# conanhujinming/flash_hash_join

Hardware: AMD Instinct MI355X
Metric: probe throughput (billion probes/sec), int64 keys, whole join (build + probe phases) per step (higher is better)
Workload: dtype int64

## Files before the change

flash_hash_join_amd/api.py:

```python
from __future__ import annotations

import ctypes
import threading
from typing import Any, Dict, Optional, Tuple

import numpy as np

from . import _lib
from ._lib import FjTimings, check

ALGO_ADAPTIVE, ALGO_SCALAR, ALGO_RADIX = 0, 1, 2
ALGO_MANY_TO_MANY = 0x10
ALGO_LEFT_OUTER = 0x20
ALGO_ANTI = 0x40
ALGO_ROW_IDS = 0x80
ALGO_FULL_OUTER = 0x100
ALGO_ALL_COPIES = 0x200
ALGO_PROBE_ORDER = 0x800
ALGO_BUILD_ORDER = 0x1000
ALGO_AGG_MIN = 0x4000
ALGO_AGG_MAX = 0x8000
ALGO_AGG_SIGNED = 0x10000
ALGO_GROUP_BY = 0x40000
ALGO_INVERSE = 0x100000
# ... 77 lines not shown
    return _ctxs[device]


def workspace_bytes(device: Optional[int] = None) -> int:
    L = _lib.load()
    return sum(int(L.fj_ctx_workspace_bytes(h)) for d, h in _ctxs.items() if device is None or d == device)


def trim_workspace(device: Optional[int] = None) -> None:
    L = _lib.load()
    for d, h in list(_ctxs.items()):
        if device is None or d == device:
            with _ctx_locks.setdefault(d, threading.RLock()):
                check(L.fj_ctx_trim(h))
    check(L.fj_ctx_trim(None))


def set_option(name: str, value: int) -> None:
    check(_lib.load().fj_set_option(name.encode(), int(value)))


def get_option(name: str) -> int:
    v = int(_lib.load().fj_get_option(name.encode()))
    if v < 0:
        raise KeyError(_lib.last_error())
    return v


def last_timings() -> Optional[dict]:
    return _last.as_dict() if _last is not None else None


def _join_host(algo: int, bloom: int, materialize: int, bk, bv, pk, return_arrays: bool):
    global _last
    L = _lib.load()
    bk, pk = _as_u64_host(bk, "build_keys"), _as_u64_host(pk, "probe_keys")
    bv = _as_u64_host(bv, "build_values") if bv is not None else None
    if bv is not None and bv.size < bk.size:
        raise ValueError(f"build_values has {bv.size} elements, build_keys has {bk.size}")
    cnt = (ctypes.c_uint64 * 3)(0, 0, 0)
    sec = ctypes.c_double(0.0)
    ok, ov = ctypes.c_void_p(), ctypes.c_void_p()
    want = bool(materialize and return_arrays)
    check(L.fj_join_host(algo, bloom, materialize, bk.ctypes.data, bv.ctypes.data if bv is not None else None, bk.size, pk.ctypes.data, pk.size,
                         cnt, ctypes.byref(sec),
                         ctypes.byref(ok) if want else None, ctypes.byref(ov) if want else None))
    t = FjTimings()
# ... 1567 lines not shown
```

flash_hash_join_amd/csrc/fj_host.h:

```cpp
#pragma once
#include "fj_internal.h"
#include "../../include/flashjoin.h"
#include "../../include/flashjoin_lab.h"

#include <algorithm>
#include <chrono>
#include <cstdarg>
#include <cstdio>
#include <cstdlib>
#include <cstring>
#include <condition_variable>
#include <functional>
#include <mutex>
#include <string>
#include <thread>
#include <vector>

struct StreamState;

namespace fjh {

int set_err(const char* fmt, ...);
fj_timings& last_timings();
#define HIPCHK(x)                                                                                          \
// ... 83 lines not shown
struct Plan { int bits = 0, npass = 0; int fan_log[4] = {0, 0, 0, 0}; int bloom_level = 0; };

struct Prepared {
    enum Form { EMPTY, LDS, HBM };
    bool valid = false;
    Form form = EMPTY;
    bool has_vals = false;
    int top_bits = 64, path = 0;
    Plan plan; u32 nparts = 0;
    size_t nb = 0; u64 g = 0;
    u64* keys = nullptr; u64* rows = nullptr; u64* vals = nullptr; void* aux = nullptr;
    u64 cap_mask = 0;
    size_t bytes = 0;
};

struct PassIter {
    int side = 0; bool has_vals = false; size_t n = 0; Plan plan; int used = 64; u32 parents = 1; u64 lbound = 0;
    u32 tile_chunks = 16; int i = 0;
    FjChunkSet prev{}; bool have_prev = false; const uint4* tiles = nullptr; const u32* ntiles = nullptr; const u32* toff = nullptr;
    FjChunkSet cs{}; u32 Gmax = 1, F = 1, appends = 1;
    size_t piece_rows = 0;
    int slot = 0, cs_base = 0;
    u32 item_tc_max = 0;
    bool want_items = false; u32 items_cap = 0; u32* part_count = nullptr; int part_count_slot = W_PART_COUNT;
    bool bloom_done = false; const FjChunkSet* bloom_build = nullptr;
    const u32* bloom_prebuilt = nullptr;
    unsigned long long* bloom_bucket_keys = nullptr;
    int save_level = 0; FjChunkSet saved{};
    u32* alloc_word = nullptr; u32* seg_word = nullptr; u32* err_word = nullptr;
    bool in_pk7 = false; u32 in_b0 = 0, in_top_shift = 0;
    bool vals_pos = false;
};

}

struct PackState {
    bool begun = false, deferred = false;
    u32 part_shift = 0;
    fjh::PassIter it;
    FjPackArgs args{};
    int nranks = 0;
};

struct StreamState {
    bool active = false;
    fjh::Plan plan; fjh::PassIter pit, bit; FjLdsJoinArgs ja{};
// ... 37 lines not shown
    u32 reserve_cus = 0;
    void* stage[3] = {nullptr, nullptr, nullptr};
    size_t stage_bytes = 0;
    bool plan_in_flight = false;
    bool slot_dirty[fjh::W_NSLOTS] = {};
    std::recursive_mutex mu;
};

namespace fjh {

#define FJ_HOOK_LOOPBACK 1
#define FJ_HOOK_INJECT_FAIL 2
#define FJ_HOOK_SPLIT_ALWAYS 4
#define FJ_HOOK_ONE_COMM 8
#define FJ_HOOK_RESERVE_ALWAYS 16
#define FJ_HOOK_EMIT_TAGGED 32
#define FJ_HOOK_EMIT_RETRY_7TH 64
struct Options {
    size_t radix_threshold = 0; int scalar_hbm_table = 0; u32 persistent_min_items = 8192; u32 plan_target_keys = FJ_PART_TARGET_KEYS;
    int bloom_variant = 0, bloom_auto = 1, bloom_auto_max_hit_bp = 2300, mat_single_pass = 1;
    int join_wide = 2;
    u32 lab_hooks = 0;
    u32 join_items_target = 2048;
    int mm_heavy_keys = 0;
    int mm_heavy_outer = 0;
    Options();
};
Options& options();

int get_buf(fj_ctx* c, int slot, size_t bytes, void** out);
int get_zeroed_buf(fj_ctx* c, int slot, size_t bytes, void** out, hipStream_t s);
int plan_npass(int bits);
void plan_passes(Plan& p, bool extra_first);
Plan make_plan(size_t nb, int top_bits, bool want_bloom = false, u64 target_override = 0);
void pass_init(PassIter& it, int side, bool has_vals, size_t n, const Plan& plan, int top_bits);
u32 pass_groups(u64 chunks, u64 rows, u32 tile_chunks, u32 F);
int pass_prepare(fj_ctx* c, PassIter& it, u32 appends, hipStream_t s);
int pass_launch(fj_ctx* c, PassIter& it, const u64* keys, const u64* vals, size_t n, hipStream_t s, int* ev_cursor);
bool bloom_stage_follows(const PassIter& it, int level);
void join_item_geometry(u64 nparts, size_t np, u64 chunk_bound, u32* tc, u64* max_items);
bool wide_join_planned(bool materialize, size_t nb, size_t np_eff, int bits);
int level_finish(fj_ctx* c, PassIter& it, bool final_level, hipStream_t s);
int pass_complete(fj_ctx* c, PassIter& it, hipStream_t s);
int bloom_stage(fj_ctx* c, PassIter& it, hipStream_t s);
int run_passes(fj_ctx* c, PassIter& it, const u64* keys, const u64* vals, hipStream_t s, FjChunkSet* out, int* ev_cursor);
int clear_plan_scalars(fj_ctx* c, hipStream_t s);
void begin_plan(fj_ctx* c);
void end_plan(fj_ctx* c);
void drop_pending(fj_ctx* c);
int begin_step(fj_ctx* c, const char* who);
int read_scalars(fj_ctx* c, hipStream_t s);
float ev_ms(fj_ctx* c, int a, int b);
void plan_timings(fj_ctx* c, const Plan& plan, u64 partitions, int evc, fj_timings* t);
int stamps_begin(unsigned long long** dbg, hipStream_t s);
int stamps_report(const char* label, const unsigned long long* dbg, u32 nitems, hipStream_t s);

int emit_pending(fj_ctx* c, u64* d_ok, u64* d_ov, size_t cap, hipStream_t s, fj_timings* t);
int radix_join_tail(fj_ctx* c, int materialize, FjLdsJoinArgs& ja, const Plan& plan, size_t np, const PassIter& pit, hipStream_t s,
                    fj_timings* t, int evc, u64* out_count, bool* lds_full, int top_bits, SingleOut* so = nullptr);

int join_outer(fj_ctx* c, int mode, bool use_radix, const u64* bk, const u64* bv, size_t nb, const u64* pk, size_t np, int top_bits,
               hipStream_t s, fj_timings* t, u64* out_count, u64* d_ok, u64* d_ov, bool rid = false);
int join_full(fj_ctx* c, bool use_radix, const u64* bk, const u64* bv, size_t nb, const u64* pk, size_t np, int top_bits,
// ... 36 lines not shown
```

flash_hash_join_amd/csrc/fj_internal.h:

```cpp
#pragma once
#include "fj_common.h"

#define FJ_ERR_POOL 1u
#define FJ_ERR_LDS_FULL 2u
#define FJ_STAT_DUPS 4u
#define FJ_STAT_RETRY 8u
#define FJ_STAT_EMIT_RETRY 16u
#define FJ_ERR_VARIANT 32u
#define FJ_BLOOM_HDR_MAGIC 0xB100F000u
#define FJ_STAT_TOOBIG 64u
#define FJ_ERR_OUTCAP 128u
#define FJ_ITEM_RETRY 0xFFFFFFFFu
#define FJ_ITEM_TOOBIG 0xFFFFFFFEu

struct FjPartArgs {
    const u64* in_keys;
    const u64* in_vals;
    const u32* in_list;
    const u32* in_dir;
    const uint4* in_tiles;
    const u32* in_ntiles;
    u64 n_flat;
    u32 parent0;
    u64* out_keys;
// ... 94 lines not shown
    u32 nsplit;
    const uint4* items;
    const u32* nitems_dev;
    u32 items_cap;
    u32* part_count;
    unsigned long long* total;
    u32* err;
    const u64* out_off;
    u64* out_keys;
    u64* out_vals;
    unsigned long long* out_cursor;
    u64 out_capacity;
    u32 retry_only;
    u32 mark_toobig;
    u32 want_dups;
    u32 dedup;
    const u64* orig_vals;
    u32 avg_build_keys;
    unsigned long long* dbg;
    u32 dbg_flags;
    u32 row_ids;
};
hipError_t fj_launch_lds_join(const FjLdsJoinArgs& a, bool materialize, hipStream_t s, u32* next_item = nullptr,
                              u32 persistent_min_items = 8192);
hipError_t fj_launch_emit_single(const FjLdsJoinArgs& a, hipStream_t s, u32* next_item);
#define FJ_WIDE_MAXSRC 16u
struct FjWideArgs {
    const u32* toff; u32 part_lo, part_hi;
    const unsigned char* base; u32 nsrc, bits, mid_bytes;
    u32 group_log;
    u32 max_units;
    u32 pmask;
    u64 offs_off[FJ_WIDE_MAXSRC], lo_off[FJ_WIDE_MAXSRC], mid_off[FJ_WIDE_MAXSRC];
};
hipError_t fj_launch_count_join_wide(const FjLdsJoinArgs& a, const FjWideArgs& w, bool dense, u32 grid, hipStream_t s);
static inline u32 fj_wide_pmask(int bits, int top_bits) { return bits <= 0 ? 0u : (bits >= 32 ? 0xFFFFFFFFu : ((1u << bits) - 1u) << (top_bits - 32 - bits)); }

hipError_t fj_launch_lds_join_retry(const FjLdsJoinArgs& a, hipStream_t s);
hipError_t fj_launch_lds_emit_retry(const FjLdsJoinArgs& a, hipStream_t s, bool only_marked = true);

hipError_t fj_launch_sample_hits(const FjChunkSet& build, const u64* pk, u64 np, u32 nsamples, u32 shift32, u32 pmask,
                                 unsigned long long* hits, hipStream_t s);

#define FJ_MM_INNER 0
#define FJ_MM_LEFT 1
#define FJ_MM_FULL 2
struct FjMmOuterArgs {
// ... 152 lines not shown
```

flash_hash_join_amd/csrc/fj_join.hip:

```cpp
#include "fj_lds_table_dev.h"

namespace {

constexpr u32 S = FJ_LDS_SLOTS;

struct JoinHdr {
    u32 cnt, has_empty, cursor, claimed, full, ovf;
    u32 pad[2];
    u64 empty_val;
    u64 pad2;
};

constexpr u32 NGRP = S / FJ_LDS_GROUP;
__device__ __forceinline__ void lds_groups(u64 key, u32& g1, u32& g2) {
    const u32 w = FJ_HW2(key);
    g1 = (w & (NGRP - 1)) * FJ_LDS_GROUP;
    g2 = ((w >> 11) & (NGRP - 1)) * FJ_LDS_GROUP;
}

__device__ __forceinline__ u32 lds_tag(u32 w2) { const u32 t = w2 >> 24; return t ? t : 1u; }
__device__ __forceinline__ u32 tag_zero_bytes(u32 t) {
    const u32 y = (t & 0x7F7F7F7Fu) + 0x7F7F7F7Fu;
    return ~(y | t | 0x7F7F7F7Fu);
}
// ... 784 lines not shown
                            const u64 ok = __ballot((okm >> (h + i)) & 1u);
                            wave_hits += (u32)__popcll(ok & ((hit & ~ise) | (ise & he)));
                        }
                    }
                    if (!parked) park();
                }
            }
        }
        if (!parked) park();
        if (lane == 0 && wave_hits) atomicAdd(&hdr->cnt, wave_hits);
        __syncthreads();
        if (lvn) load_build(bmn, 0, nbbn); else bok = 0;
        if (tid == 0) {
            const u32 cnt = (lv && !full) ? hdr->cnt : 0u;
            if (full) atomicOr(a.err, FJ_STAT_RETRY);
            a.part_count[d.item] = full ? FJ_ITEM_RETRY : cnt;
            if (cnt) atomicAdd(a.total, (unsigned long long)cnt);
        }
        if (dn.item >= nitems) break;
        __syncthreads();
        reset_table();
        __syncthreads();
        d = dn; buf ^= 1;
    }
}

struct EkHdr { u32 has_empty, nstash, full, dups, cursor, novf, cur2[2]; u64 empty_val; u64 gb2[2]; u64 pad; u64 stash[CK_STASH]; u64 stash_val[CK_STASH]; };

template <int NT, bool DEDUP, bool SINGLE = false, bool RID = false>
__global__ __launch_bounds__(NT, 4) void fj_emit_join_persistent(FjLdsJoinArgs a, u32* __restrict__ next_item) {
    static_assert(!(SINGLE && DEDUP), "the single-pass form serves unique build keys");
    extern __shared__ __attribute__((aligned(16))) unsigned char smem[];
    EkHdr* hdr = reinterpret_cast<EkHdr*>(smem);
    u64* tkeys = reinterpret_cast<u64*>(smem + sizeof(EkHdr));
    u64* tvals = tkeys + S;
    u32* pm0 = reinterpret_cast<u32*>(tvals + S);
    u32* bm0 = pm0 + 2 * JP_META;
    u32* s_next = bm0 + 2 * JB_META;
    u32* bits = s_next + 4;
    u64* ovf = reinterpret_cast<u64*>(bits + S / 32);
    u32 tid = threadIdx.x;
    const u32 lane = tid & 63, wave_s = (u32)__builtin_amdgcn_readfirstlane((int)(threadIdx.x >> 6));
    auto fresh_tid = [&]() -> u32 {
        u32 t;
        asm volatile("v_mbcnt_lo_u32_b32 %0, -1, 0\n\tv_mbcnt_hi_u32_b32 %0, -1, %0\n\tv_lshl_add_u32 %0, %1, 6, %0" : "=&v"(t) : "s"(wave_s));
        return t;
// ... 811 lines not shown
    const u64 stride = (u64)gridDim.x * blockDim.x;
    for (u64 i = (u64)blockIdx.x * blockDim.x + threadIdx.x; i < n; i += stride) {
        keys[i] = (first + i + 1) * FJ_GOLDEN;
        vals[i] = first + i;
    }
}
__global__ void fj_gen_probe_kernel(u64* __restrict__ keys, u64 first, u64 n, u64 B, u64 seed, u32 hit_bp,
                                    unsigned long long* __restrict__ expected) {
    const u64 stride = (u64)gridDim.x * blockDim.x;
    u32 hits = 0;
    for (u64 i = (u64)blockIdx.x * blockDim.x + threadIdx.x; i < n; i += stride) {
        const u64 j = first + i;
        const u64 r = 1 + fj_mix(seed, j) % B;
        const bool hit = (fj_mix(seed ^ 1ull, j) % 10000ull) < hit_bp;
        keys[i] = (r + (hit ? 0ull : B)) * FJ_GOLDEN;
        hits += hit ? 1u : 0u;
    }
    hits = fj_wave_sum(hits);
    if ((threadIdx.x & 63) == 0 && hits) atomicAdd(expected, (unsigned long long)hits);
}

}

hipError_t fj_launch_lds_join(const FjLdsJoinArgs& a, bool materialize, hipStream_t s, u32* next_item, u32 persistent_min_items) {
    const u32 nb = a.items ? a.items_cap : a.nparts * a.nsplit;
    if (materialize) {
        if (a.row_ids && (!a.dedup || a.orig_vals)) return hipErrorInvalidValue;
        if (a.build.list && a.probe.list && a.items && next_item && nb >= persistent_min_items && !a.dbg && !(a.dbg_flags & ~8u)) {
            const u32 ldsp = sizeof(EkHdr) + 2 * S * 8 + 2 * (JP_META + JB_META) * 4 + 16 + S / 8 + CK_OVF * 8;
            auto pk = a.row_ids ? fj_emit_join_persistent<1024, true, false, true>
                                : a.dedup ? fj_emit_join_persistent<1024, true> : fj_emit_join_persistent<1024, false>;
            hipError_t e = fj_set_max_lds_once(reinterpret_cast<const void*>(pk), ldsp);
            if (e != hipSuccess) return e;
            const u32 grid = nb < 256 ? nb : 256;
            hipLaunchKernelGGL(pk, dim3(grid), dim3(1024), ldsp, s, a, next_item);
            return hipGetLastError();
        }
        if (a.row_ids) return fj_launch_lds_emit_retry(a, s, false);
        const u32 lds = sizeof(JoinHdr) + 2 * S * 8 + S + S / 2 + (JP_META + JB_META) * 4;
        auto kern = (a.build.list && a.probe.list) ? fj_lds_join_kernel<true, 1024, true> : fj_lds_join_kernel<true, 1024, false>;
        hipError_t e = fj_set_max_lds_once(reinterpret_cast<const void*>(kern), lds);
        if (e != hipSuccess) return e;
        hipLaunchKernelGGL(kern, dim3(nb), dim3(1024), lds, s, a);
    } else {
        const u32 lds = sizeof(CkHdr) + S * 8 + (JP_META + JB_META) * 4 + S / 8 + CK_OVF * 8;
        const bool lists = a.build.list && a.probe.list;
        if (lists && next_item && nb >= persistent_min_items && !a.dbg && !a.dbg_flags) {
            const u32 ldsp = sizeof(CkHdr) + S * 8 + 2 * (JP_META + JB_META) * 4 + 16 + S / 8 + CK_OVF * 8;
            auto pk = fj_count_join_persistent<512>;
            hipError_t e = fj_set_max_lds_once(reinterpret_cast<const void*>(pk), ldsp);
            if (e != hipSuccess) return e;
            const u32 grid = nb < 512 ? nb : 512;
            hipLaunchKernelGGL(pk, dim3(grid), dim3(512), ldsp, s, a, next_item);
            return hipGetLastError();
        }
        auto kern = lists ? fj_count_join_kernel<512, true> : fj_count_join_kernel<512, false>;
        hipError_t e = fj_set_max_lds_once(reinterpret_cast<const void*>(kern), lds);
        if (e != hipSuccess) return e;
        hipLaunchKernelGGL(kern, dim3(nb), dim3(512), lds, s, a);
    }
    return hipGetLastError();
}

hipError_t fj_launch_emit_single(const FjLdsJoinArgs& a, hipStream_t s, u32* next_item) {
    if (!a.build.list || !a.probe.list || !a.items || !next_item || !a.out_cursor || a.dedup || !a.build.vals || (a.row_ids && !a.probe.vals))
        return hipErrorInvalidValue;
    const u32 nb = a.items_cap;
    const u32 ldsp = sizeof(EkHdr) + 2 * S * 8 + 2 * (JP_META + JB_META) * 4 + 16 + S / 8 + CK_OVF * 8;
    auto pk = a.row_ids ? fj_emit_join_persistent<1024, false, true, true> : fj_emit_join_persistent<1024, false, true>;
// ... 154 lines not shown
```

flash_hash_join_amd/csrc/fj_joins.hip:

```cpp
#include "fj_host.h"

namespace fjh {

static int skew_side(fj_ctx* c, PassIter& it, int side, bool vals, const FjChunkSet& in, const std::vector<u32>& off, u64 chunks, int S, int bits_left,
                     int slot, int tiles_slot, u32* d_nt, hipStream_t s);

int emit_pending(fj_ctx* c, u64* d_ok, u64* d_ov, size_t cap, hipStream_t s, fj_timings* t) {
    Pending& pd = c->pend;
    if (!pd.valid) return set_err("fj_emit_pairs: no counted materialising join is pending on this context");
    if (pd.count > cap) return set_err("fj_emit_pairs: output capacity %zu < %llu pairs", cap, (unsigned long long)pd.count);
    if (pd.count > 0 && (((uintptr_t)d_ok | (uintptr_t)d_ov) & 7)) return set_err("output buffers must be 8-byte aligned");
    HIPCHK(hipEventRecord(c->ev[E_EMIT0], s));
    if (pd.count > 0) {
        void* p;
        if (pd.kind == Pending::LDS) {
            if (pd.lds.row_ids) {
                pd.lds.dedup = 1; pd.lds.orig_vals = nullptr;
            } else if (pd.has_dups) {
                if (get_buf(c, W_ROWIDX, pd.nb * 8, &p)) return 1;
                u64* rowidx = (u64*)p;
                HIPCHK(fj_launch_iota(rowidx, pd.nb, s));
                HIPCHK(hipMemsetAsync(&c->d_sc->alloc[0], 0, sizeof(c->d_sc->alloc) + sizeof(c->d_sc->seg_counter), s));
                PassIter bit;
                pass_init(bit, 0, true, pd.nb, make_plan(pd.nb, pd.top_bits), pd.top_bits);
// ... 316 lines not shown
        const u32 grid = std::min<u32>(nitems, c->num_cus);
        HIPCHK(fj_launch_count_join_wide(jw, wa, false, grid, s));
        if (jw.dbg) {
            std::vector<unsigned long long> h(4096 * 8);
            HIPCHK(hipStreamSynchronize(s));
            HIPCHK(hipMemcpy(h.data(), jw.dbg, h.size() * 8, hipMemcpyDeviceToHost));
            double acc[8] = {0, 0, 0, 0, 0, 0, 0, 0};
            for (u32 g = 0; g < grid && g < 4096; ++g) for (int i = 0; i < 8; ++i) acc[i] += (double)h[g * 8 + i] * 0.01;
            u32 nit = 0;
            HIPCHK(hipMemcpy(&nit, jw.nitems_dev, 4, hipMemcpyDeviceToHost));
            const double per = (double)std::min<u32>(grid, 4096) * ((double)nit / grid);
            fprintf(stderr, "[FJ_WIDE_STAMPS] us per item (thread 0): rotate+requests %.3f  claim_issue+zero %.3f  barB %.3f  probe %.3f  resolve+park %.3f  barA %.3f  stores %.3f\n",
                    acc[0] / per, acc[5] / per, acc[6] / per, acc[1] / per, acc[2] / per, acc[3] / per, acc[4] / per);
            for (int ph = 0; ph < 3; ++ph) {
                fprintf(stderr, "[FJ_WIDE_STAMPS] wave 0..15, %s:", ph == 0 ? "requests + claims issued + probe" : ph == 1 ? "claims resolved + park (to barrier A)" : "stores (barrier A to B)");
                for (int w = 0; w < 16; ++w) {
                    double sacc = 0;
                    for (u32 g = 0; g < grid && g < 256; ++g) sacc += (double)h[2048 * 8 + g * 64 + w * 4 + ph] * 0.01;
                    fprintf(stderr, " %.2f", sacc / ((double)std::min<u32>(grid, 256) * ((double)nit / grid)));
                }
                fprintf(stderr, "\n");
            }
        }
    } else
    HIPCHK(fj_launch_lds_join(ja, false, s, &c->d_sc->next_item, options().persistent_min_items));
    if (ja.dbg) { if (stamps_report("FJ_JOIN_STAMPS", ja.dbg, nitems, s)) return 1; ja.dbg = nullptr; }
    HIPCHK(hipEventRecord(c->ev[E_JOIN], s));
    if (read_scalars(c, s)) return 1;
    t->lds_retries = 0;
    if ((c->h_sc->err & FJ_STAT_RETRY) && !(c->h_sc->err & (FJ_ERR_POOL | FJ_ERR_LDS_FULL))) {
        ja.retry_only = 1; ja.mark_toobig = ja.items ? 1u : 0u;
        HIPCHK(fj_launch_lds_join_retry(ja, s));
        ja.retry_only = 0;
        HIPCHK(hipEventRecord(c->ev[E_JOIN], s));
        if (read_scalars(c, s)) return 1;
        t->lds_retries = 1;
        if ((c->h_sc->err & FJ_STAT_TOOBIG) && !(c->h_sc->err & (FJ_ERR_POOL | FJ_ERR_LDS_FULL))) {
            bool ok = false; u32 redone = 0;
            if (skew_join(c, ja, plan, top_bits, nitems, pit.slot, materialize, s, &ok, &redone, &c->pend)) return 1;
            HIPCHK(hipEventRecord(c->ev[E_JOIN], s));
            if (read_scalars(c, s)) return 1;
            if (ok) t->lds_retries = 1 + (int)redone;
            else c->h_sc->err |= FJ_ERR_LDS_FULL;
        }
    }
    if (c->h_sc->err & FJ_ERR_POOL) return set_err("internal error: chunk pool exhausted during a partition pass");
    end_plan(c);
    plan_timings(c, plan, ja.nparts, evc, t);
// ... 22 lines not shown
    pass_init(bit, 0, materialize != 0, nb, plan, top_bits);
    bit.vals_pos = rid;
    int evc = 0;
    if (plan.bloom_level > 0) bit.save_level = plan.bloom_level;
    if (run_passes(c, bit, bk, (materialize && !rid) ? bv : nullptr, s, &ja.build, nullptr)) return 1;
    HIPCHK(hipEventRecord(c->ev[E_BUILD], s));
    Plan pplan = plan;
    if (bloom == 2) {
        const u32 nsamp = FJ_SAMPLE_KEYS;
        HIPCHK(fj_launch_sample_hits(ja.build, pk, np, nsamp, (u32)(top_bits - 32 - plan.bits), (1u << plan.bits) - 1u, &c->d_sc->sample_hits, s));
        HIPCHK(hipMemcpyAsync(&c->h_sc->sample_hits, &c->d_sc->sample_hits, sizeof(unsigned long long), hipMemcpyDeviceToHost, s));
        HIPCHK(hipStreamSynchronize(s));
        const u32 hit_bp = (u32)(c->h_sc->sample_hits * 10000ull / nsamp);
        t->sampled_hit_bp = (int)hit_bp;
        if (hit_bp > (u32)options().bloom_auto_max_hit_bp) { pplan = make_plan(nb, top_bits, false); plan.bloom_level = 0; plan.npass = pplan.npass; }
    }
    pass_init(pit, 1, rid, np, pplan, top_bits);
    pit.vals_pos = rid;
    pit.want_items = true;
    {
        size_t np_eff = np;
        if (plan.bloom_level > 0) np_eff = (size_t)((double)np * (t->sampled_hit_bp >= 0 ? std::min(10000, t->sampled_hit_bp + 1000) : 1500) / 10000.0);
        if (wide_join_planned(materialize != 0, nb, np_eff, plan.bits)) pit.item_tc_max = 32;
    }
    if (plan.bloom_level > 0) pit.bloom_build = &bit.saved;
    if (run_passes(c, pit, pk, nullptr, s, &ja.probe, &evc)) return 1;
    HIPCHK(hipEventRecord(c->ev[E_PPART], s));
    ja.avg_build_keys = (u32)std::min<u64>(0xFFFFFFFFu, (u64)nb >> plan.bits);
    ja.row_ids = rid ? 1u : 0u;
    if (radix_join_tail(c, materialize, ja, plan, np, pit, s, t, evc, out_count, lds_full, top_bits, so)) return 1;
    if (c->pend.valid) { c->pend.bk = bk; c->pend.bv = bv; c->pend.nb = nb; c->pend.top_bits = top_bits; }
    return 0;
}

static int mm_tile_join(fj_ctx* c, const FjLdsJoinArgs& ja, u32 nitems, int materialize, hipStream_t s, Pending* pend,
                        int outer = FJ_MM_INNER, const FjMmOuterArgs* oa = nullptr) {
    u32 nlive = 0;
    std::vector<u32> pc(nitems), boff((size_t)ja.build.nb + 1);
    std::vector<uint4> items(nitems);
    HIPCHK(hipMemcpyAsync(&nlive, ja.nitems_dev, 4, hipMemcpyDeviceToHost, s));
    HIPCHK(hipMemcpyAsync(pc.data(), ja.part_count, (size_t)nitems * 4, hipMemcpyDeviceToHost, s));
    HIPCHK(hipMemcpyAsync(items.data(), ja.items, (size_t)nitems * sizeof(uint4), hipMemcpyDeviceToHost, s));
    HIPCHK(hipMemcpyAsync(boff.data(), ja.build.boff, boff.size() * 4, hipMemcpyDeviceToHost, s));
    HIPCHK(hipStreamSynchronize(s));
    if (nlive > nitems) nlive = nitems;
    std::vector<uint4> tiles, big;
// ... 586 lines not shown
```

flash_hash_join_amd/csrc/fj_plan.hip:

```cpp
#include "fj_host.h"

namespace fjh {

namespace { thread_local std::string g_err; thread_local fj_timings g_last; }

int set_err(const char* fmt, ...) {
    char buf[1024];
    va_list ap; va_start(ap, fmt); vsnprintf(buf, sizeof buf, fmt, ap); va_end(ap);
    g_err = buf;
    return 1;
}
fj_timings& last_timings() { return g_last; }

Options& options() { static Options o; return o; }
static int set_option_value(Options& o, const char* name, long long value);
Options::Options() {
    static const char* const legacy[] = {"FJ_RADIX_THRESHOLD", "FJ_SCALAR_HBM_TABLE", "FJ_BLOOM_AUTO", "FJ_BLOOM_AUTO_MAX_HIT_BP", "FJ_BLOOM_VARIANT", "FJ_PLAN_TARGET_KEYS",
                                         "FJ_MAT_SINGLE_PASS", "FJ_PERSISTENT_MIN_ITEMS", "FJ_JOIN_ITEMS_TARGET", "FJ_JOIN_WIDE", "FJ_DIST_LOOPBACK", "FJ_DIST_INJECT_FAIL",
                                         "FJ_DIST_RESERVE_ALWAYS", "FJ_DIST_SPLIT_ALWAYS", "FJ_DIST_ONE_COMM", "FJ_EMIT_TAGGED"};
    for (const char* name : legacy)
        if (getenv(name)) fprintf(stderr, "flash_hash_join_amd: the environment variable %s is no longer read (use FJ_OPTIONS=\"name=value,...\" or fj_set_option; see include/flashjoin.h)\n", name);
    const char* e = getenv("FJ_OPTIONS");
    if (!e) return;
    std::string str(e);
// ... 129 lines not shown
        a.in_keys = it.prev.keys; a.in_vals = it.prev.vals; a.in_list = it.prev.list; a.in_dir = it.prev.dir;
        a.in_tiles = it.tiles; a.in_ntiles = it.ntiles; a.n_flat = 0;
    } else {
        a.in_keys = keys; a.in_vals = vals; a.in_list = nullptr; a.in_dir = nullptr; a.in_tiles = nullptr; a.in_ntiles = nullptr; a.n_flat = n;
        a.vals_pos = it.has_vals && it.vals_pos ? 1u : 0u;
        G = std::min(G, pass_groups((n + FJ_CHUNK - 1) / FJ_CHUNK, n, it.tile_chunks, it.F));
    }
    a.parent0 = 0;
    a.out_keys = cs.keys; a.out_vals = cs.vals; a.out_dir = cs.dir; a.out_rel = cs.rel; a.seg_off = cs.seg_off;
    a.bchunks = cs.bchunks; a.alloc = cs.alloc; a.seg_counter = it.seg_word ? it.seg_word : &c->d_sc->seg_counter[it.side * 4 + it.i];
    a.cap_chunks = cs.cap; a.max_segs = cs.max_segs;
    a.err = it.err_word ? it.err_word : &c->d_sc->err;
    if (it.have_prev && it.in_pk7) { a.in_pk7 = 1; a.in_b0 = it.in_b0; a.in_top_shift = it.in_top_shift; }
    a.shift = (u32)it.used; a.fan_log = (u32)it.plan.fan_log[it.i]; a.slab = fj_slab_for(it.appends); a.run_log = cs.run_log; a.side = (u32)it.side;
    const int line_log = (it.has_vals && it.F > 256) ? 3 : 4;
    if (ev_cursor) HIPCHK(hipEventRecord(c->ev[E_PK0 + 2 * (*ev_cursor)], s));
    HIPCHK(fj_launch_partition(a, it.has_vals, line_log, G, s));
    if (ev_cursor) { HIPCHK(hipEventRecord(c->ev[E_PK0 + 2 * (*ev_cursor) + 1], s)); ++*ev_cursor; }
    return 0;
}

bool bloom_stage_follows(const PassIter& it, int level) { return it.plan.bloom_level == level && it.bloom_build && !it.bloom_done; }

void join_item_geometry(u64 nparts, size_t np, u64 chunk_bound, u32* tc, u64* max_items) {
    const u64 pchunks = (np + FJ_CHUNK - 1) / FJ_CHUNK;
    const u64 bound = std::max<u64>(chunk_bound, pchunks);
    const u64 avg = std::max<u64>(1, bound / nparts);
    u64 want = 1;
    const u64 target_items = options().join_items_target;
    if (nparts < target_items) want = std::min<u64>((target_items + nparts - 1) / nparts, std::max<u64>(1, (pchunks / nparts) / 32));
    *tc = (u32)(want > 1 ? std::max<u64>(8, (avg * 9 / 8 + want - 1) / want) : std::max<u64>(512, 4 * avg));
    *max_items = bound / *tc + nparts + 1;
}

bool wide_join_planned(bool materialize, size_t nb, size_t np_eff, int bits) {
    if (materialize || bits <= 0 || options().join_wide == 0) return false;
    if (options().join_wide == 1) return true;
    return np_eff <= 3 * nb;
}

int level_finish(fj_ctx* c, PassIter& it, bool final_level, hipStream_t s) {
    const FjChunkSet& cs = it.cs;
    u32 tc = 0; u64 max_tiles = 0; u32* zero_tail = nullptr;
    if (bloom_stage_follows(it, it.i)) tc = fj_bloom_tile_chunks();
    else if (!final_level) tc = fj_partition_tile_chunks((u32)it.plan.fan_log[it.i], it.has_vals);
    else if (it.want_items) {
        join_item_geometry(cs.nb, it.n, it.lbound, &tc, &max_tiles);
        if (it.item_tc_max && tc > it.item_tc_max) { tc = it.item_tc_max; max_tiles = std::max<u64>(it.lbound, (it.n + FJ_CHUNK - 1) / FJ_CHUNK) / tc + cs.nb + 1; }
    }
    if (tc && !max_tiles) max_tiles = it.lbound / tc + cs.nb + 1;
    if (max_tiles >= (1ull << 31)) return set_err("internal error: tile table too large");
    u32* toff = nullptr; uint4* tiles = nullptr;
    void* p;
    if (tc) {
        if (get_buf(c, it.cs_base + W_TOFF, ((size_t)cs.nb + 1) * 4, &p)) return 1; toff = (u32*)p;
        if (get_buf(c, it.cs_base + W_TILES, max_tiles * sizeof(uint4), &p)) return 1; tiles = (uint4*)p;
        if (final_level) {
            if (get_buf(c, it.part_count_slot, (size_t)max_tiles * 4, &p)) return 1;
            it.part_count = zero_tail = (u32*)p; it.items_cap = (u32)max_tiles;
        }
    }
    HIPCHK(fj_launch_group(cs, tc, toff, tiles, (u32)max_tiles, zero_tail, s));
    it.tiles = tiles; it.ntiles = toff ? toff + cs.nb : nullptr; it.toff = toff;
    return 0;
}

int pass_complete(fj_ctx* c, PassIter& it, hipStream_t s) {
    const FjChunkSet& cs = it.cs;
    it.lbound = it.n / FJ_CHUNK + 1 + (u64)(it.Gmax + it.parents) * it.F * it.appends;
    ++it.i;
// ... 116 lines not shown
        for (int j = 1; j <= 5; ++j) acc[j] += (double)(r[j] - r[j - 1]) * 0.01;
        if (r[0] < tmin) tmin = r[0];
        if (r[5] > tmax) tmax = r[5];
        ++n;
    }
    if (n == 0) n = 1;
    fprintf(stderr, "[%s] items=%d  meta+init=%.2f  build=%.2f  buildsync=%.2f  probe=%.2f  fin=%.2f us (means); first 4096 items span %.1f us\n",
            label, n, acc[1] / n, acc[2] / n, acc[3] / n, acc[4] / n, acc[5] / n, (double)(tmax - tmin) * 0.01);
    return 0;
}

static int set_option_value(Options& o, const char* name, long long value) {
    if (!strcmp(name, "radix_threshold")) { if (value < 0) return set_err("fj_set_option: radix_threshold must be >= 0"); o.radix_threshold = (size_t)value; return 0; }
    if (!strcmp(name, "scalar_hbm_table")) { o.scalar_hbm_table = value != 0; return 0; }
    if (!strcmp(name, "plan_target_keys")) { if (value < 16 || value > (long long)FJ_PART_TARGET_KEYS) return set_err("fj_set_option: plan_target_keys must be 16..%u", FJ_PART_TARGET_KEYS); o.plan_target_keys = (u32)value; return 0; }
    if (!strcmp(name, "bloom_auto")) { o.bloom_auto = value != 0; return 0; }
    if (!strcmp(name, "mat_single_pass")) { o.mat_single_pass = value != 0; return 0; }
    if (!strcmp(name, "bloom_auto_max_hit_bp")) { if (value < 0 || value > 10000) return set_err("fj_set_option: bloom_auto_max_hit_bp must be 0..10000"); o.bloom_auto_max_hit_bp = (int)value; return 0; }
    if (!strcmp(name, "bloom_variant")) { if (value < 0 || value > 2) return set_err("fj_set_option: bloom_variant must be 0..2"); o.bloom_variant = (int)value; return 0; }
    if (!strcmp(name, "join_wide")) { if (value < 0 || value > 2) return set_err("fj_set_option: join_wide must be 0..2"); o.join_wide = (int)value; return 0; }
    if (!strcmp(name, "persistent_min_items")) { if (value < 0) return set_err("fj_set_option: persistent_min_items must be >= 0"); o.persistent_min_items = (u32)std::min<long long>(value, 0xFFFFFFFFll); return 0; }
    if (!strcmp(name, "lab_hooks")) { if (value < 0 || value > 0xFFFF) return set_err("fj_set_option: lab_hooks is a mask of FJ_HOOK_* bits"); o.lab_hooks = (u32)value; return 0; }
    if (!strcmp(name, "join_items_target")) { if (value < 1 || value > (1 << 20)) return set_err("fj_set_option: join_items_target must be 1..1048576"); o.join_items_target = (u32)value; return 0; }
    if (!strcmp(name, "mm_heavy_keys")) { if (value < 0 || value > 1) return set_err("fj_set_option: mm_heavy_keys must be 0 or 1"); o.mm_heavy_keys = (int)value; return 0; }
    if (!strcmp(name, "mm_heavy_outer")) { if (value < 0 || value > 1) return set_err("fj_set_option: mm_heavy_outer must be 0 or 1"); o.mm_heavy_outer = (int)value; return 0; }
    return set_err("fj_set_option: unknown option '%s'", name);
}

}
using namespace fjh;

void fj_set_error_string(const char* msg) { fjh::g_err = msg ? msg : ""; }

extern "C" {

const char* fj_last_error(void) { return fjh::g_err.c_str(); }
const char* fj_version(void) { return "flash_hash_join_amd 0.6 (gfx950)"; }
int fj_abi_version(void) { return FJ_ABI_VERSION; }

int fj_set_option(const char* name, long long value) {
    if (!name) return set_err("fj_set_option: null name");
    return fjh::set_option_value(options(), name, value);
}

long long fj_get_option(const char* name) {
    const Options& o = options();
    if (name && !strcmp(name, "radix_threshold")) return (long long)o.radix_threshold;
    if (name && !strcmp(name, "scalar_hbm_table")) return o.scalar_hbm_table;
    if (name && !strcmp(name, "persistent_min_items")) return o.persistent_min_items;
    if (name && !strcmp(name, "join_wide")) return o.join_wide;
    if (name && !strcmp(name, "plan_target_keys")) return o.plan_target_keys;
    if (name && !strcmp(name, "bloom_variant")) return o.bloom_variant;
    if (name && !strcmp(name, "bloom_auto")) return o.bloom_auto;
    if (name && !strcmp(name, "mat_single_pass")) return o.mat_single_pass;
    if (name && !strcmp(name, "bloom_auto_max_hit_bp")) return o.bloom_auto_max_hit_bp;
    if (name && !strcmp(name, "lab_hooks")) return o.lab_hooks;
    if (name && !strcmp(name, "join_items_target")) return o.join_items_target;
    if (name && !strcmp(name, "mm_heavy_keys")) return o.mm_heavy_keys;
    if (name && !strcmp(name, "mm_heavy_outer")) return o.mm_heavy_outer;
    set_err("fj_get_option: unknown option '%s'", name ? name : "(null)");
    return -1;
}

uint64_t fj_key_mix64(uint64_t key) { return fj_key_mix(key); }
uint64_t fj_key_unmix64(uint64_t mixed) { return fj_key_unmix(mixed); }

int fj_device_count(void) {
    int n = 0;
    if (hipGetDeviceCount(&n) != hipSuccess) return 0;
    return n;
}

int fj_initialize(void) {
    int n = 0;
    hipError_t e = hipGetDeviceCount(&n);
    if (e != hipSuccess || n <= 0) return set_err("fj_initialize: no usable HIP device (%s)", e == hipSuccess ? "device count is 0" : hipGetErrorString(e));
    return 0;
}

fj_ctx* fj_ctx_create(int device) {
// ... 122 lines not shown
```

Measured before the change: 115.9.

## Add grouped count-join kernel that builds each partition table once per item run

Adds a count-join kernel that walks contiguous runs of probe items belonging to the same partition and builds the LDS cuckoo table once per run, so it is not rebuilt for every item. The planner can now split probe work into more, smaller items when grouping is enabled (join_group_items, join_group_min_chunks), which gives better load balance without repeated build-side loads. This is on by default (join_group_log=-1, which falls back to static even division of items across 512 blocks). The risk is that static run assignment replaces the atomic-counter persistent scheduler and can cause imbalance.

Measured after the change: 116.5 (median of 2 runs). About the same (+0.5%).

```diff
diff --git a/flash_hash_join_amd/api.py b/flash_hash_join_amd/api.py
--- a/flash_hash_join_amd/api.py
+++ b/flash_hash_join_amd/api.py
@@ -123,7 +123,7 @@
 
 def get_option(name: str) -> int:
     v = int(_lib.load().fj_get_option(name.encode()))
-    if v < 0:
+    if v < 0 and _lib.last_error():
         raise KeyError(_lib.last_error())
     return v
 
diff --git a/flash_hash_join_amd/csrc/fj_host.h b/flash_hash_join_amd/csrc/fj_host.h
--- a/flash_hash_join_amd/csrc/fj_host.h
+++ b/flash_hash_join_amd/csrc/fj_host.h
@@ -129,6 +129,8 @@
     size_t piece_rows = 0;
     int slot = 0, cs_base = 0;
     u32 item_tc_max = 0;
+    int group_mode = 0;
+    bool items_grouped = false;
     bool want_items = false; u32 items_cap = 0; u32* part_count = nullptr; int part_count_slot = W_PART_COUNT;
     bool bloom_done = false; const FjChunkSet* bloom_build = nullptr;
     const u32* bloom_prebuilt = nullptr;
@@ -212,6 +214,9 @@
     int join_wide = 2;
     u32 lab_hooks = 0;
     u32 join_items_target = 2048;
+    int join_group_log = -1;
+    u32 join_group_items = 16384;
+    u32 join_group_min_chunks = 8;
     int mm_heavy_keys = 0;
     int mm_heavy_outer = 0;
     Options();
@@ -228,7 +233,7 @@
 int pass_prepare(fj_ctx* c, PassIter& it, u32 appends, hipStream_t s);
 int pass_launch(fj_ctx* c, PassIter& it, const u64* keys, const u64* vals, size_t n, hipStream_t s, int* ev_cursor);
 bool bloom_stage_follows(const PassIter& it, int level);
-void join_item_geometry(u64 nparts, size_t np, u64 chunk_bound, u32* tc, u64* max_items);
+void join_item_geometry(u64 nparts, size_t np, u64 chunk_bound, u32* tc, u64* max_items, int group_mode = 0, bool* grouped = nullptr);
 bool wide_join_planned(bool materialize, size_t nb, size_t np_eff, int bits);
 int level_finish(fj_ctx* c, PassIter& it, bool final_level, hipStream_t s);
 int pass_complete(fj_ctx* c, PassIter& it, hipStream_t s);
diff --git a/flash_hash_join_amd/csrc/fj_internal.h b/flash_hash_join_amd/csrc/fj_internal.h
--- a/flash_hash_join_amd/csrc/fj_internal.h
+++ b/flash_hash_join_amd/csrc/fj_internal.h
@@ -140,7 +140,7 @@
     u32 row_ids;
 };
 hipError_t fj_launch_lds_join(const FjLdsJoinArgs& a, bool materialize, hipStream_t s, u32* next_item = nullptr,
-                              u32 persistent_min_items = 8192);
+                              u32 persistent_min_items = 8192, int group_run_len = -1, const u32* item_off = nullptr);
 hipError_t fj_launch_emit_single(const FjLdsJoinArgs& a, hipStream_t s, u32* next_item);
 #define FJ_WIDE_MAXSRC 16u
 struct FjWideArgs {
diff --git a/flash_hash_join_amd/csrc/fj_join.hip b/flash_hash_join_amd/csrc/fj_join.hip
--- a/flash_hash_join_amd/csrc/fj_join.hip
+++ b/flash_hash_join_amd/csrc/fj_join.hip
@@ -830,6 +830,231 @@
         reset_table();
         __syncthreads();
         d = dn; buf ^= 1;
+    }
+}
+
+template <int NT>
+__global__ __launch_bounds__(NT, 4) void fj_count_join_grouped(FjLdsJoinArgs a, const u32* __restrict__ item_off, u32 run_len) {
+    extern __shared__ __attribute__((aligned(16))) unsigned char smem[];
+    CkHdr* hdr = reinterpret_cast<CkHdr*>(smem);
+    u64* tkeys = reinterpret_cast<u64*>(smem + sizeof(CkHdr));
+    u32* pm0 = reinterpret_cast<u32*>(tkeys + S);
+    u32* bm0 = pm0 + 2 * JP_META;
+    u32* bits = bm0 + 2 * JB_META + 4;
+    u64* ovf = reinterpret_cast<u64*>(bits + S / 32);
+    const u32 tid = threadIdx.x, lane = tid & 63;
+    const u32 nitems = *a.nitems_dev;
+    const u32 G = gridDim.x;
+    constexpr u32 CPL = NT / (FJ_CHUNK / 2), CPR = 4 * CPL, BKPT = 4096 / NT;
+    static_assert(JP_META <= NT && JB_META <= NT, "one staged list entry per thread");
+
+    auto run_bounds = [&](u32 r, u32& lo, u32& hi) {
+        if (run_len) {
+            const u64 l = (u64)r * run_len;
+            lo = l < nitems ? (u32)l : nitems;
+            hi = nitems - lo < run_len ? nitems : lo + run_len;
+        } else {
+            const u32 q = nitems / G, rem = nitems % G;
+            lo = r < G ? r * q + (r < rem ? r : rem) : nitems;
+            hi = r < G ? lo + q + (r < rem ? 1u : 0u) : nitems;
+        }
+        lo = __builtin_amdgcn_readfirstlane(lo); hi = __builtin_amdgcn_readfirstlane(hi);
+    };
+    struct Desc { u32 item, nit, b0, nbc, s_lo, s_hi; };
+    auto describe = [&](u32 item, u32 run_hi) -> Desc {
+        Desc d; d.item = item; d.nit = 0; d.b0 = 0; d.nbc = 0; d.s_lo = 0; d.s_hi = 0;
+        if (item >= run_hi || item >= nitems) { d.item = nitems; return d; }
+        const uint4 it = a.items[item];
+        const u32 pend = item_off[it.z + 1];
+        u32 last = (run_hi < pend ? run_hi : pend) - 1;
+        if (last < item) last = item;
+        const uint4 itl = a.items[last];
+        const u32 b0 = a.build.boff[it.z], b1 = a.build.boff[it.z + 1];
+        d.nit = __builtin_amdgcn_readfirstlane(last - item + 1);
+        d.b0 = __builtin_amdgcn_readfirstlane(b0); d.nbc = __builtin_amdgcn_readfirstlane(b1 - b0);
+        d.s_lo = __builtin_amdgcn_readfirstlane(it.x); d.s_hi = __builtin_amdgcn_readfirstlane(itl.x + itl.y);
+        return d;
+    };
+    auto live = [&](const Desc& d) { return d.item < nitems && d.nbc > 0 && d.s_lo < d.s_hi; };
+
+    u64 bk[BKPT];
+    u32 bok = 0;
+    auto load_build = [&](const u32* bm, u32 c0, u32 nbb) {
+        bok = 0;
+#pragma unroll
+        for (u32 j = 0; j < BKPT; ++j) {
+            const u32 kidx = j * NT + tid, c = c0 + (kidx >> FJ_CHUNK_LOG), off = kidx & (FJ_CHUNK - 1);
+            const u32 e = bm[c < nbb ? c : nbb - 1];
+            bk[j] = a.build.keys[(u64)FJ_LIST_ID(e) * FJ_CHUNK + off];
+            bok |= (c < nbb && off < FJ_LIST_CNT(e) ? 1u : 0u) << j;
+        }
+    };
+    auto load_round = [&](const u32* pm, u32 r, u32 nbatch, u64 (&kk)[8], u32& okm) {
+        okm = 0;
+#pragma unroll
+        for (int u = 0; u < 4; ++u) {
+            const u32 c = r * CPR + u * CPL + tid / (FJ_CHUNK / 2), off = (tid % (FJ_CHUNK / 2)) * 2;
+            const u32 e = pm[c < nbatch ? c : nbatch - 1], cnt = c < nbatch ? FJ_LIST_CNT(e) : 0;
+            const u64x2 q = *reinterpret_cast<const u64x2*>(a.probe.keys + (u64)FJ_LIST_ID(e) * FJ_CHUNK + off);
+            kk[2 * u] = q.x; kk[2 * u + 1] = q.y;
+            okm |= ((off < cnt ? 1u : 0u) | (off + 1 < cnt ? 2u : 0u)) << (2 * u);
+        }
+    };
+    auto reset_table = [&]() {
+        for (u32 i = tid; i < S; i += NT) tkeys[i] = FJ_EMPTY_KEY;
+        if (tid < S / 32) bits[tid] = 0;
+        if (tid == 0) { hdr->cnt = 0; hdr->has_empty = 0; hdr->nstash = 0; hdr->full = 0; hdr->dups = 0; hdr->empties = 0; hdr->novf = 0; }
+    };
+
+    u32 run = blockIdx.x, run_lo, run_hi;
+    run_bounds(run, run_lo, run_hi);
+    Desc d = describe(run_lo, run_hi);
+    if (d.item >= nitems) return;
+    u32 buf = 0;
+    {
+        const bool lv = live(d);
+        const u32 nb0 = (d.s_hi - d.s_lo) < JP_META ? (d.s_hi - d.s_lo) : JP_META;
+        if (lv && tid < nb0) pm0[tid] = a.probe.list[d.s_lo + tid];
+        const u32 nbb0 = d.nbc < JB_META ? d.nbc : JB_META;
+        if (lv && tid < nbb0) bm0[tid] = a.build.list[d.b0 + tid];
+        reset_table();
+        __syncthreads();
+        if (lv) load_build(bm0, 0, nbb0);
+    }
+
+    for (;;) {
+        u32* pm = pm0 + buf * JP_META; u32* bm = bm0 + buf * JB_META;
+        u32* pmn = pm0 + (buf ^ 1) * JP_META; u32* bmn = bm0 + (buf ^ 1) * JB_META;
+        const bool lv = live(d);
+        u64 ka[8], kb[8];
+        u32 oka = 0, okb = 0;
+        u32 nbatch = (d.s_hi - d.s_lo) < JP_META ? (d.s_hi - d.s_lo) : JP_META;
+        u32 nrounds = (nbatch + CPR - 1) / CPR;
+        if (lv) {
+            load_round(pm, 0, nbatch, ka, oka);
+            if (nrounds > 1) load_round(pm, 1, nbatch, kb, okb);
+            u32 nbb = d.nbc < JB_META ? d.nbc : JB_META;
+            for (u32 bb = 0; bb < d.nbc; bb += JB_META) {
+                if (bb) {
+                    nbb = (d.nbc - bb) < JB_META ? (d.nbc - bb) : JB_META;
+                    __syncthreads();
+                    if (tid < nbb) bm[tid] = a.build.list[d.b0 + bb + tid];
+                    __syncthreads();
+                }
+                for (u32 c0 = 0; c0 < nbb; c0 += 16) {
+                    if (bb | c0) load_build(bm, c0, nbb);
+#pragma unroll
+                    for (u32 j = 0; j < BKPT; ++j) {
+                        if (bok & (1u << j)) {
+                            if (bk[j] == FJ_EMPTY_KEY) { hdr->has_empty = 1; if (a.want_dups && atomicAdd(&hdr->empties, 1u) > 0) hdr->dups = 1; }
+                            else cuckoo_claim(tkeys, bits, ovf, hdr, bk[j]);
+                        }
+                    }
+                }
+            }
+        }
+        __syncthreads();
+        if (lv) cuckoo_finish<NT>(tkeys, ovf, hdr, tid);
+        __syncthreads();
+        u32 nitem = d.item + d.nit, nhi = run_hi;
+        if (nitem >= run_hi) {
+            if (run_len) { run += G; run_bounds(run, nitem, nhi); }
+            else nitem = nhi = nitems;
+        }
+        const Desc dn = describe(nitem, nhi);
+        const bool lvn = live(dn);
+        const u32 nbn = (dn.s_hi - dn.s_lo) < JP_META ? (dn.s_hi - dn.s_lo) : JP_META;
+        const u32 nbbn = dn.nbc < JB_META ? dn.nbc : JB_META;
+        u32 mp = 0, mb = 0;
+        if (lvn && tid < nbn) mp = a.probe.list[dn.s_lo + tid];
+        if (lvn && tid < nbbn) mb = a.build.list[dn.b0 + tid];
+        bool parked = false;
+        auto park = [&]() {
+            if (tid < nbn) pmn[tid] = mp;
+            if (tid < nbbn) bmn[tid] = mb;
+            parked = true;
+        };
+
+        u32 wave_hits = 0;
+        bool full = false;
+        if (lv) {
+            full = hdr->full != 0;
+            const u64 he = hdr->has_empty ? ~0ull : 0ull;
+            const u32 nstash = hdr->nstash < CK_STASH ? hdr->nstash : CK_STASH;
+            if (a.want_dups && !full) {
+                for (u32 sl = tid; sl < S; sl += NT) {
+                    const u64 key = tkeys[sl];
+                    if (key == FJ_EMPTY_KEY) continue;
+                    const u32 w = FJ_HW2(key), l1 = w & (S - 1), l2 = (w >> 13) & (S - 1);
+                    const u32 other = sl == l1 ? l2 : l1;
+                    if (other != sl && tkeys[other] == key) hdr->dups = 1;
+                    for (u32 si = 0; si < nstash; ++si) if (hdr->stash[si] == key) hdr->dups = 1;
+                }
+                for (u32 si = tid; si < nstash; si += NT)
+                    for (u32 sj = si + 1; sj < nstash; ++sj) if (hdr->stash[si] == hdr->stash[sj]) hdr->dups = 1;
+                __syncthreads();
+                if (tid == 0 && hdr->dups) atomicOr(a.err, FJ_STAT_DUPS);
+            }
+            if (!full) for (u32 pb = d.s_lo; pb < d.s_hi; pb += JP_META) {
+                if (pb != d.s_lo) {
+                    nbatch = (d.s_hi - pb) < JP_META ? (d.s_hi - pb) : JP_META;
+                    __syncthreads();
+                    if (tid < nbatch) pm[tid] = a.probe.list[pb + tid];
+                    __syncthreads();
+                    nrounds = (nbatch + CPR - 1) / CPR;
+                    load_round(pm, 0, nbatch, ka, oka);
+                    if (nrounds > 1) load_round(pm, 1, nbatch, kb, okb);
+                }
+                for (u32 r = 0; r < nrounds; ++r) {
+                    u64 k[8];
+#pragma unroll
+                    for (int i = 0; i < 8; ++i) { k[i] = ka[i]; ka[i] = kb[i]; }
+                    const u32 okm = oka;
+                    oka = okb;
+                    if (r + 2 < nrounds) load_round(pm, r + 2, nbatch, kb, okb);
+#pragma unroll
+                    for (int h = 0; h < 8; h += 4) {
+                        u64 c1[4], c2[4];
+#pragma unroll
+                        for (int i = 0; i < 4; ++i) {
+                            const u32 w = FJ_HW2(k[h + i]);
+                            c1[i] = tkeys[w & (S - 1)];
+                            c2[i] = tkeys[(w >> 13) & (S - 1)];
+                        }
+                        __builtin_amdgcn_sched_barrier(0);
+#pragma unroll
+                        for (int i = 0; i < 4; ++i) {
+                            u64 hit = __ballot(c1[i] == k[h + i]) | __ballot(c2[i] == k[h + i]);
+                            if (nstash) {
+                                bool f = false;
+                                for (u32 si = 0; si < nstash; ++si) f |= hdr->stash[si] == k[h + i];
+                                hit |= __ballot(f);
+                            }
+                            const u64 ise = __ballot(k[h + i] == FJ_EMPTY_KEY);
+                            const u64 ok = __ballot((okm >> (h + i)) & 1u);
+                            wave_hits += (u32)__popcll(ok & ((hit & ~ise) | (ise & he)));
+                        }
+                    }
+                    if (!parked) park();
+                }
+            }
+        }
+        if (!parked) park();
+        if (lane == 0 && wave_hits) atomicAdd(&hdr->cnt, wave_hits);
+        __syncthreads();
+        if (lvn) load_build(bmn, 0, nbbn); else bok = 0;
+        if (tid == 0) {
+            const u32 cnt = (lv && !full) ? hdr->cnt : 0u;
+            if (full) atomicOr(a.err, FJ_STAT_RETRY);
+            a.part_count[d.item] = full ? FJ_ITEM_RETRY : cnt;
+            if (cnt) atomicAdd(a.total, (unsigned long long)cnt);
+        }
+        for (u32 i = 1 + tid; i < d.nit; i += NT) a.part_count[d.item + i] = full ? FJ_ITEM_RETRY : 0u;
+        if (dn.item >= nitems) break;
+        __syncthreads();
+        reset_table();
+        __syncthreads();
+        d = dn; run_hi = nhi; buf ^= 1;
     }
 }
 
@@ -1687,7 +1912,8 @@
 
 }
 
-hipError_t fj_launch_lds_join(const FjLdsJoinArgs& a, bool materialize, hipStream_t s, u32* next_item, u32 persistent_min_items) {
+hipError_t fj_launch_lds_join(const FjLdsJoinArgs& a, bool materialize, hipStream_t s, u32* next_item, u32 persistent_min_items,
+                              int group_run_len, const u32* item_off) {
     const u32 nb = a.items ? a.items_cap : a.nparts * a.nsplit;
     if (materialize) {
         if (a.row_ids && (!a.dedup || a.orig_vals)) return hipErrorInvalidValue;
@@ -1710,6 +1936,16 @@
     } else {
         const u32 lds = sizeof(CkHdr) + S * 8 + (JP_META + JB_META) * 4 + S / 8 + CK_OVF * 8;
         const bool lists = a.build.list && a.probe.list;
+        if (lists && a.items && item_off && group_run_len >= 0 && !a.dbg && !a.dbg_flags) {
+            const u32 ldsp = sizeof(CkHdr) + S * 8 + 2 * (JP_META + JB_META) * 4 + 16 + S / 8 + CK_OVF * 8;
+            auto gk = fj_count_join_grouped<512>;
+            hipError_t e = fj_set_max_lds_once(reinterpret_cast<const void*>(gk), ldsp);
+            if (e != hipSuccess) return e;
+            const u32 nruns = group_run_len ? (nb + (u32)group_run_len - 1) / (u32)group_run_len : nb;
+            const u32 grid = nruns < 512 ? nruns : 512;
+            hipLaunchKernelGGL(gk, dim3(grid), dim3(512), ldsp, s, a, item_off, (u32)group_run_len);
+            return hipGetLastError();
+        }
         if (lists && next_item && nb >= persistent_min_items && !a.dbg && !a.dbg_flags) {
             const u32 ldsp = sizeof(CkHdr) + S * 8 + 2 * (JP_META + JB_META) * 4 + 16 + S / 8 + CK_OVF * 8;
             auto pk = fj_count_join_persistent<512>;
diff --git a/flash_hash_join_amd/csrc/fj_joins.hip b/flash_hash_join_amd/csrc/fj_joins.hip
--- a/flash_hash_join_amd/csrc/fj_joins.hip
+++ b/flash_hash_join_amd/csrc/fj_joins.hip
@@ -362,8 +362,12 @@
                 fprintf(stderr, "\n");
             }
         }
-    } else
-    HIPCHK(fj_launch_lds_join(ja, false, s, &c->d_sc->next_item, options().persistent_min_items));
+    } else {
+        int run_len = -1;
+        if (pit.items_grouped && options().join_group_log != 0 && !materialize && ja.probe.list && ja.build.list && ja.items && pit.toff)
+            run_len = options().join_group_log < 0 ? 0 : 1 << options().join_group_log;
+        HIPCHK(fj_launch_lds_join(ja, false, s, &c->d_sc->next_item, options().persistent_min_items, run_len, pit.toff));
+    }
     if (ja.dbg) { if (stamps_report("FJ_JOIN_STAMPS", ja.dbg, nitems, s)) return 1; ja.dbg = nullptr; }
     HIPCHK(hipEventRecord(c->ev[E_JOIN], s));
     if (read_scalars(c, s)) return 1;
@@ -432,6 +436,7 @@
         size_t np_eff = np;
         if (plan.bloom_level > 0) np_eff = (size_t)((double)np * (t->sampled_hit_bp >= 0 ? std::min(10000, t->sampled_hit_bp + 1000) : 1500) / 10000.0);
         if (wide_join_planned(materialize != 0, nb, np_eff, plan.bits)) pit.item_tc_max = 32;
+        else pit.group_mode = materialize ? 0 : options().join_group_log;
     }
     if (plan.bloom_level > 0) pit.bloom_build = &bit.saved;
     if (run_passes(c, pit, pk, nullptr, s, &ja.probe, &evc)) return 1;
diff --git a/flash_hash_join_amd/csrc/fj_plan.hip b/flash_hash_join_amd/csrc/fj_plan.hip
--- a/flash_hash_join_amd/csrc/fj_plan.hip
+++ b/flash_hash_join_amd/csrc/fj_plan.hip
@@ -175,15 +175,24 @@
 
 bool bloom_stage_follows(const PassIter& it, int level) { return it.plan.bloom_level == level && it.bloom_build && !it.bloom_done; }
 
-void join_item_geometry(u64 nparts, size_t np, u64 chunk_bound, u32* tc, u64* max_items) {
+void join_item_geometry(u64 nparts, size_t np, u64 chunk_bound, u32* tc, u64* max_items, int group_mode, bool* grouped) {
     const u64 pchunks = (np + FJ_CHUNK - 1) / FJ_CHUNK;
     const u64 bound = std::max<u64>(chunk_bound, pchunks);
     const u64 avg = std::max<u64>(1, bound / nparts);
     u64 want = 1;
+    bool g = false;
     const u64 target_items = options().join_items_target;
-    if (nparts < target_items) want = std::min<u64>((target_items + nparts - 1) / nparts, std::max<u64>(1, (pchunks / nparts) / 32));
+    if (nparts < target_items) {
+        const u64 full = (target_items + nparts - 1) / nparts;
+        want = std::min<u64>(full, std::max<u64>(1, (pchunks / nparts) / 32));
+        g = want > 1 && (group_mode > 0 || (group_mode < 0 && want == full));
+        if (g) want = std::min<u64>((std::max<u64>(options().join_group_items, target_items) + nparts - 1) / nparts,
+                                    std::max<u64>(1, (pchunks / nparts) / options().join_group_min_chunks));
+        g = g && want > 1;
+    }
     *tc = (u32)(want > 1 ? std::max<u64>(8, (avg * 9 / 8 + want - 1) / want) : std::max<u64>(512, 4 * avg));
     *max_items = bound / *tc + nparts + 1;
+    if (grouped) *grouped = g;
 }
 
 bool wide_join_planned(bool materialize, size_t nb, size_t np_eff, int bits) {
@@ -198,7 +207,7 @@
     if (bloom_stage_follows(it, it.i)) tc = fj_bloom_tile_chunks();
     else if (!final_level) tc = fj_partition_tile_chunks((u32)it.plan.fan_log[it.i], it.has_vals);
     else if (it.want_items) {
-        join_item_geometry(cs.nb, it.n, it.lbound, &tc, &max_tiles);
+        join_item_geometry(cs.nb, it.n, it.lbound, &tc, &max_tiles, it.item_tc_max ? 0 : it.group_mode, &it.items_grouped);
         if (it.item_tc_max && tc > it.item_tc_max) { tc = it.item_tc_max; max_tiles = std::max<u64>(it.lbound, (it.n + FJ_CHUNK - 1) / FJ_CHUNK) / tc + cs.nb + 1; }
     }
     if (tc && !max_tiles) max_tiles = it.lbound / tc + cs.nb + 1;
@@ -361,6 +370,9 @@
     if (!strcmp(name, "persistent_min_items")) { if (value < 0) return set_err("fj_set_option: persistent_min_items must be >= 0"); o.persistent_min_items = (u32)std::min<long long>(value, 0xFFFFFFFFll); return 0; }
     if (!strcmp(name, "lab_hooks")) { if (value < 0 || value > 0xFFFF) return set_err("fj_set_option: lab_hooks is a mask of FJ_HOOK_* bits"); o.lab_hooks = (u32)value; return 0; }
     if (!strcmp(name, "join_items_target")) { if (value < 1 || value > (1 << 20)) return set_err("fj_set_option: join_items_target must be 1..1048576"); o.join_items_target = (u32)value; return 0; }
+    if (!strcmp(name, "join_group_log")) { if (value < -1 || value > 6) return set_err("fj_set_option: join_group_log must be -1..6"); o.join_group_log = (int)value; return 0; }
+    if (!strcmp(name, "join_group_items")) { if (value < 1 || value > (1 << 20)) return set_err("fj_set_option: join_group_items must be 1..1048576"); o.join_group_items = (u32)value; return 0; }
+    if (!strcmp(name, "join_group_min_chunks")) { if (value < 1 || value > 4096) return set_err("fj_set_option: join_group_min_chunks must be 1..4096"); o.join_group_min_chunks = (u32)value; return 0; }
     if (!strcmp(name, "mm_heavy_keys")) { if (value < 0 || value > 1) return set_err("fj_set_option: mm_heavy_keys must be 0 or 1"); o.mm_heavy_keys = (int)value; return 0; }
     if (!strcmp(name, "mm_heavy_outer")) { if (value < 0 || value > 1) return set_err("fj_set_option: mm_heavy_outer must be 0 or 1"); o.mm_heavy_outer = (int)value; return 0; }
     return set_err("fj_set_option: unknown option '%s'", name);
@@ -384,6 +396,7 @@
 
 long long fj_get_option(const char* name) {
     const Options& o = options();
+    fjh::g_err.clear();
     if (name && !strcmp(name, "radix_threshold")) return (long long)o.radix_threshold;
     if (name && !strcmp(name, "scalar_hbm_table")) return o.scalar_hbm_table;
     if (name && !strcmp(name, "persistent_min_items")) return o.persistent_min_items;
@@ -395,6 +408,9 @@
     if (name && !strcmp(name, "bloom_auto_max_hit_bp")) return o.bloom_auto_max_hit_bp;
     if (name && !strcmp(name, "lab_hooks")) return o.lab_hooks;
     if (name && !strcmp(name, "join_items_target")) return o.join_items_target;
+    if (name && !strcmp(name, "join_group_log")) return o.join_group_log;
+    if (name && !strcmp(name, "join_group_items")) return o.join_group_items;
+    if (name && !strcmp(name, "join_group_min_chunks")) return o.join_group_min_chunks;
     if (name && !strcmp(name, "mm_heavy_keys")) return o.mm_heavy_keys;
     if (name && !strcmp(name, "mm_heavy_outer")) return o.mm_heavy_outer;
     set_err("fj_get_option: unknown option '%s'", name ? name : "(null)");
```
